# philip-bl/dctn

Hardware: AMD Instinct MI355X
Metric: EPS-contraction windows/sec (fwd+bwd) (higher is better)
Workload: dtype bf16; 1 GPU; cfg2 EPS[(3,4)]+linear bf16 B1024/GPU; parallelism=dp1

## Files before the change

dctn_amd/csrc/eps_mfma.hip:

```cpp
#include "common.h"

#include <cstdlib>
#include <type_traits>

typedef __attribute__((ext_vector_type(8))) __bf16 bf16x8;
typedef __attribute__((ext_vector_type(16))) float f32x16;
typedef __attribute__((ext_vector_type(8))) float f32x8;
typedef __attribute__((ext_vector_type(2))) int int2v;
typedef __attribute__((ext_vector_type(4))) int int4v;
typedef __attribute__((ext_vector_type(2))) float f32x2;

namespace {

constexpr int ilog2(int v) { return v <= 1 ? 0 : 1 + ilog2(v >> 1); }

template <typename S> __device__ __forceinline__ float to_f32(S v) { return (float)v; }

__device__ __forceinline__ float half_sum(float v) {
  const int iv = __float_as_int(v);
  const int2v r = __builtin_amdgcn_permlane32_swap(iv, iv, false, false);
  return __int_as_float(r[0]) + __int_as_float(r[1]);
}

__device__ __forceinline__ void swap_halves(float& a, float& b) {
// ... 20 lines not shown
}

typedef short s16x4 __attribute__((ext_vector_type(4)));
typedef short s16x8 __attribute__((ext_vector_type(8)));
constexpr int LROW = 32;
struct TrLane {
  int wr[4];
  int rd_lo, rd_hi;
};
__device__ __forceinline__ TrLane tr_lane(int lane) {
  TrLane t;
#pragma unroll
  for (int c = 0; c < 4; ++c) t.wr[c] = lane * LROW + (((c + (lane >> 1)) & 3) << 3);
  const int g = lane >> 4, q = (lane >> 2) & 3, pp = lane & 3;
  const int lc = 2 * (g & 1) + (pp >> 1), half = pp & 1;
  const int row = 8 * (g >> 1) + q;
  t.rd_lo = row * LROW + (((lc + (row >> 1)) & 3) << 3) + 4 * half;
  t.rd_hi = (row + 4) * LROW + (((lc + ((row + 4) >> 1)) & 3) << 3) + 4 * half;
  return t;
}
__device__ __forceinline__ bf16x8 tr_frag(const short* tile, int ks, const TrLane& t) {
  typedef __attribute__((address_space(3))) s16x4 lds_s16x4;
  const s16x4 lo = __builtin_amdgcn_ds_read_tr16_b64_v4i16((lds_s16x4*)(tile + t.rd_lo + ks * 16 * LROW));
  const s16x4 hi = __builtin_amdgcn_ds_read_tr16_b64_v4i16((lds_s16x4*)(tile + t.rd_hi + ks * 16 * LROW));
  const s16x8 v = {lo[0], lo[1], lo[2], lo[3], hi[0], hi[1], hi[2], hi[3]};
  return __builtin_bit_cast(bf16x8, v);
}

struct FastDiv {
  unsigned M, s1, s2;
};
__device__ __forceinline__ unsigned fdiv(unsigned n, const FastDiv& d) {
  const unsigned t = __umulhi(d.M, n);
  return (t + ((n - t) >> d.s1)) >> d.s2;
}

#define MFMA_MAXN 16
struct MfmaP {
  int C, B, K, O, Ho, Wo;
  int P;
  int npg;
  int spc, nchunks;
  unsigned foffb[MFMA_MAXN];
  unsigned rowoffb[MFMA_MAXN];
  unsigned s1b, s2b, s3b, s4b;
  unsigned x_bytes;
  unsigned o_bytes, o_s1b;
  FastDiv div_wo;
  int rowvec_ok;
  int vec_ok;
  int Cout;
  unsigned hw_rowb, hw_bytes;
  int ncb;
  int opts;
#ifdef DCTN_STAMPS
  unsigned long long* stamps;
#endif
};

#ifdef DCTN_STAMPS
#define DCTN_STAMP(P, SLOT)                                                                      \
  do {                                                                                           \
    __builtin_amdgcn_sched_barrier(0);                                                           \
    unsigned long long t_;                                                                       \
    asm volatile("s_memrealtime %0\n\ts_waitcnt lgkmcnt(0)" : "=s"(t_)::"memory");               \
    if ((P).stamps && threadIdx.x == 0) (P).stamps[(long long)blockIdx.x * 8 + (SLOT)] = t_;     \
    __builtin_amdgcn_sched_barrier(0);                                                           \
  } while (0)
static unsigned long long* g_stamps = nullptr;
void dctn_stamps_set(unsigned long long* p) { g_stamps = p; }
__device__ unsigned long long* g_dev_stamps = nullptr;
void dctn_reduce_stamps_set(unsigned long long* p) { (void)hipMemcpyToSymbol(HIP_SYMBOL(g_dev_stamps), &p, sizeof(p)); }
#define DCTN_STAMP_T(P, SLOT, TID)                                                              \
  do {                                                                                           \
    __builtin_amdgcn_sched_barrier(0);                                                           \
    unsigned long long t_;                                                                       \
    asm volatile("s_memrealtime %0\n\ts_waitcnt lgkmcnt(0)" : "=s"(t_)::"memory");               \
    if ((P).stamps && threadIdx.x == (TID)) (P).stamps[(long long)blockIdx.x * 8 + (SLOT)] = t_;  \
    __builtin_amdgcn_sched_barrier(0);                                                           \
  } while (0)
#define DCTN_STAMP_ROLE_ROW 1024
#define DCTN_STAMP_R(P, SLOT)                                                                    \
  do {                                                                                           \
    __builtin_amdgcn_sched_barrier(0);                                                           \
    unsigned long long t_;                                                                       \
    asm volatile("s_memrealtime %0\n\ts_waitcnt lgkmcnt(0)" : "=s"(t_)::"memory");               \
    if ((P).stamps && threadIdx.x == 64 * 8)                                                     \
      (P).stamps[(long long)(DCTN_STAMP_ROLE_ROW + blockIdx.x) * 8 + (SLOT)] = t_;               \
    __builtin_amdgcn_sched_barrier(0);                                                           \
  } while (0)
#define DCTN_STAMP_G(SLOT)                                                                       \
  do {                                                                                           \
    __builtin_amdgcn_sched_barrier(0);                                                           \
    unsigned long long t_;                                                                       \
    asm volatile("s_memrealtime %0\n\ts_waitcnt lgkmcnt(0)" : "=s"(t_)::"memory");               \
    if (g_dev_stamps && threadIdx.x == 0) g_dev_stamps[(long long)blockIdx.x * 8 + (SLOT)] = t_;  \
    __builtin_amdgcn_sched_barrier(0);                                                           \
  } while (0)
#else
#define DCTN_STAMP(P, SLOT) do { } while (0)
#define DCTN_STAMP_T(P, SLOT, TID) do { } while (0)
#define DCTN_STAMP_G(SLOT) do { } while (0)
#define DCTN_STAMP_R(P, SLOT) do { } while (0)
#endif

typedef __attribute__((ext_vector_type(4))) unsigned u32x4;
typedef __attribute__((ext_vector_type(2))) unsigned u32x2;
typedef __attribute__((ext_vector_type(2))) __bf16 bf16x2;

__device__ __forceinline__ __amdgpu_buffer_rsrc_t make_rsrc(const void* ptr, unsigned bytes) {
  return __builtin_amdgcn_make_buffer_rsrc(const_cast<void*>(ptr), 0, (int)bytes, 0x00020000);
}

template <typename S, int N, bool VEC, int ROWS>
struct RawWindow {
  u32x4 row[ROWS > 0 ? ROWS : 1];
  unsigned v[(ROWS == 0 && VEC) ? N * (int)(sizeof(S) / 2) : 1];
  unsigned e[(ROWS == 0 && !VEC) ? 2 * N : 1];
};

template <typename S, int N, bool VEC, int ROWS>
__device__ __forceinline__ void issue_window(__amdgpu_buffer_rsrc_t rs, unsigned voff, unsigned soff,
                                             const MfmaP& p, RawWindow<S, N, VEC, ROWS>& raw) {
  if constexpr (ROWS > 0) {
#pragma unroll
    for (int rw = 0; rw < ROWS; ++rw)
      raw.row[rw] = __builtin_amdgcn_raw_buffer_load_b128(rs, voff, soff + p.rowoffb[rw], 0);
  } else if constexpr (VEC) {
#pragma unroll
    for (int n = 0; n < N; ++n) {
      if constexpr (sizeof(S) == 2) {
        raw.v[n] = __builtin_amdgcn_raw_buffer_load_b32(rs, voff, soff + p.foffb[n], 0);
      } else {
        const u32x2 t = __builtin_amdgcn_raw_buffer_load_b64(rs, voff, soff + p.foffb[n], 0);
        raw.v[2 * n] = t.x;
        raw.v[2 * n + 1] = t.y;
      }
    }
  } else {
#pragma unroll
    for (int n = 0; n < N; ++n)
#pragma unroll
      for (int q = 0; q < 2; ++q) {
        if constexpr (sizeof(S) == 2)
          raw.e[2 * n + q] = (unsigned)(unsigned short)__builtin_amdgcn_raw_buffer_load_b16(
              rs, voff, soff + p.foffb[n] + q * p.s4b, 0);
        else
          raw.e[2 * n + q] = __builtin_amdgcn_raw_buffer_load_b32(rs, voff, soff + p.foffb[n] + q * p.s4b, 0);
      }
  }
}

template <typename S, int N, bool VEC, int ROWS>
__device__ __forceinline__ void unpack_window(const RawWindow<S, N, VEC, ROWS>& raw, float (&xv)[N][2]) {
  if constexpr (ROWS > 0) {
    constexpr int KK = N / ROWS;
// ... 94 lines not shown
template <typename S, int OP, bool VEC>
__device__ __forceinline__ void store_row(__amdgpu_buffer_rsrc_t rs, unsigned voff, unsigned soff, int O,
                                          const float (&v)[OP]) {
  constexpr int DW = RawRow<S, OP>::DW;
  if constexpr (VEC) {
    unsigned d[DW];
#pragma unroll
    for (int i = 0; i < DW; ++i)
      d[i] = sizeof(S) == 2 ? pack_bf16(v[2 * i], v[2 * i + 1]) : __float_as_uint(v[i * (OP / DW)]);
    if constexpr (DW == 1) {
      __builtin_amdgcn_raw_buffer_store_b32(d[0], rs, voff, soff, 0);
    } else if constexpr (DW == 2) {
      __builtin_amdgcn_raw_buffer_store_b64(u32x2{d[0], d[1]}, rs, voff, soff, 0);
    } else {
#pragma unroll
      for (int i = 0; i < DW / 4; ++i)
        __builtin_amdgcn_raw_buffer_store_b128(u32x4{d[4 * i], d[4 * i + 1], d[4 * i + 2], d[4 * i + 3]}, rs, voff,
                                               soff + 16u * i, 0);
    }
  } else {
#pragma unroll
    for (int o = 0; o < OP; ++o)
      if (o < O) {
        if constexpr (sizeof(S) == 2)
          __builtin_amdgcn_raw_buffer_store_b16((unsigned short)(pack_bf16(v[o], 0.f) & 0xffffu), rs, voff,
                                                soff + 2u * o, 0);
        else
          __builtin_amdgcn_raw_buffer_store_b32(__float_as_uint(v[o]), rs, voff, soff + 4u * o, 0);
      }
  }
}

struct WaveJob {
  int b0, b1;
  unsigned voff_x;
  unsigned voff_o;
  int pos;
  bool valid;
};
__device__ __forceinline__ WaveJob wave_job(const MfmaP& p, int waves_per_block, int esz, bool grouped = false) {
  const int nb = gridDim.x;
  const int vb = (nb % 8 == 0) ? (int)(blockIdx.x % 8) * (nb / 8) + (int)(blockIdx.x / 8) : (int)blockIdx.x;
  const int wave = __builtin_amdgcn_readfirstlane(vb * waves_per_block + (int)(threadIdx.x >> 6));
  int chunk = wave / p.npg, pg = wave - chunk * p.npg;
  if (grouped) {
    const int cb = vb / p.npg;
    pg = vb - cb * p.npg;
    chunk = __builtin_amdgcn_readfirstlane(cb * waves_per_block + (int)(threadIdx.x >> 6));
    if (cb >= p.ncb) chunk = p.nchunks;
  }
  WaveJob j;
  j.b0 = chunk < p.nchunks ? chunk * p.spc : 0;
  j.b1 = chunk < p.nchunks ? (j.b0 + p.spc < p.B ? j.b0 + p.spc : p.B) : 0;
  j.pos = pg * 64 + (int)(threadIdx.x & 63);
  j.valid = j.pos < p.P;
  const unsigned pu = j.valid ? (unsigned)j.pos : 0u;
  const unsigned ho = fdiv(pu, p.div_wo), wo = pu - ho * (unsigned)p.Wo;
  j.voff_x = j.valid ? ho * p.s2b + wo * p.s3b : p.x_bytes;
  j.voff_o = j.valid ? pu * (unsigned)(p.O * esz) : p.o_bytes;
  return j;
}

template <int N0>
__device__ __forceinline__ void build_p0(const float (*xv)[2], bf16x8 (&X)[(1 << N0) / 16],
                                         bf16x8 (&Y)[(1 << N0) / 16]) {
  constexpr int KS = (1 << N0) / 16;
  const f32x2 x1 = {xv[N0 - 1][0], xv[N0 - 1][1]}, x2 = {xv[N0 - 2][0], xv[N0 - 2][1]};
  const f32x2 m01 = bmul2(xv[N0 - 3][0], x2), m23 = bmul2(xv[N0 - 3][1], x2);
  const f32x2 lo[4] = {bmul2(m01[0], x1), bmul2(m01[1], x1), bmul2(m23[0], x1), bmul2(m23[1], x1)};
#pragma unroll
  for (int s = 0; s < KS; ++s) {
    float hi = 1.f;
#pragma unroll
    for (int t = 0; t < N0 - 4; ++t) hi = t == 0 ? xv[N0 - 5][s & 1] : hi * xv[N0 - 5 - t][(s >> t) & 1];
    const f32x2 x4 = {xv[N0 - 4][0], xv[N0 - 4][1]};
    const f32x2 h = N0 > 4 ? bmul2(hi, x4) : x4;
    int4v rx, ry;
#pragma unroll
    for (int i = 0; i < 4; ++i) {
      const f32x2 a = bmul2(h[0], lo[i]), b = bmul2(h[1], lo[i]);
      rx[i] = (int)pack_bf16(a[0], a[1]);
      ry[i] = (int)pack_bf16(b[0], b[1]);
    }
    X[s] = __builtin_bit_cast(bf16x8, rx);
    Y[s] = __builtin_bit_cast(bf16x8, ry);
  }
}

template <typename S, int N0, int N1, int OP, bool XVEC, bool OVEC, int ROWS>
__global__ __launch_bounds__(256) __attribute__((amdgpu_waves_per_eu(OP <= 4 ? 4 : 2))) void eps_fwd_q2reg_k(const S* __restrict__ x,
                                                       const S* __restrict__ core,
                                                       S* __restrict__ out, double* __restrict__ stats, MfmaP p) {
  constexpr int N = N0 + N1, A = 1 << N0, BN = 1 << N1, KS = A / 16, MT = BN * OP / 32;
  constexpr int LOGO = ilog2(OP);
  static_assert(MT >= 1 && KS >= 1, "tile too small");
  constexpr int TOT = A * BN * OP, PER = TOT / 256;
  static_assert(TOT % 256 == 0, "core staging assumes a multiple of 256 elements");
  __shared__ __attribute__((aligned(16))) bf16_t cs[TOT];
  const int tid = threadIdx.x, lane = tid & 63;
  DCTN_STAMP(p, 0);
  const WaveJob job = wave_job(p, 4, (int)sizeof(S));
  const __amdgpu_buffer_rsrc_t rs_x = make_rsrc(x, p.x_bytes), rs_o = make_rsrc(out, p.o_bytes);
  RawWindow<S, N, XVEC, ROWS> raw;
  if (job.b0 < job.b1) issue_window<S, N, XVEC, ROWS>(rs_x, job.voff_x, (unsigned)job.b0 * p.s1b, p, raw);
  {
    S tmp[PER];
// ... 281 lines not shown
    f32x4v hd = {0.f, 0.f, 0.f, 0.f};
#pragma unroll
    for (int ks = 0; ks < HK; ++ks) {
      const bf16x8 fb = *reinterpret_cast<const bf16x8*>(brd + 32 * ks);
      hd = __builtin_amdgcn_mfma_f32_16x16x32_bf16(wf[ks], fb, hd, 0, 0, 0);
    }
    wave_lds_sync();
    {
      const int sl = lane & 15, cb = 4 * (lane >> 4);
      if (sl < g1 - g0) {
#pragma unroll
        for (int v = 0; v < 4; ++v) hsum[grp & 1][sl][cb + v][wv] = hd[v];
      }
    }
    DCTN_STAMP(p, 3);
    __syncthreads();
    for (int e = tid; e < (g1 - g0) * p.Cout; e += (int)blockDim.x) {
      const int sl = e / p.Cout, c = e - sl * p.Cout;
      float t = (float)bias[c];
      for (int w = 0; w < nwv; ++w) t += hsum[grp & 1][sl][c][w];
      logits[(long long)(g0 + sl) * p.Cout + c] = (bf16_t)t;
    }
  }
  DCTN_STAMP(p, 4);
}

constexpr int HEADT_WAVES = 16;
constexpr int HEADT_GS = 4;
constexpr int HEADT_MAXKS = 6;
constexpr int headt_pitch(int F) { return (F + 31) / 32 * 32 + 8; }

template <int N0, int N1, int OP, int ROWS, bool BLK4>
__global__ __launch_bounds__(64 * HEADT_WAVES) void eps_fwd_head_q2reg_t_k(const bf16_t* __restrict__ x,
                                                                           const bf16_t* __restrict__ core,
                                                                           const bf16_t* __restrict__ hw,
                                                                           const bf16_t* __restrict__ bias,
                                                                           bf16_t* __restrict__ out,
                                                                           bf16_t* __restrict__ logits, MfmaP p) {
  typedef bf16_t S;
  typedef __attribute__((ext_vector_type(4))) float f32x4v;
  constexpr int N = N0 + N1, A = 1 << N0, BN = 1 << N1, KS = A / 16, MT = BN * OP / 32;
  constexpr int LOGO = ilog2(OP);
  constexpr int TOT = A * BN * OP;
  static_assert(OP % 2 == 0 && TOT % 4 == 0, "outputs are handled as bf16 pairs");
  __shared__ __attribute__((aligned(16))) bf16_t cs[TOT];
  __shared__ float hsum[HEADT_WAVES][HEADT_GS][16];
  __shared__ unsigned step_ctr;
  extern __shared__ __attribute__((aligned(16))) short ftile[];
  const int tid = threadIdx.x, lane = tid & 63;
  const int wv = __builtin_amdgcn_readfirstlane(tid >> 6);
  const int b0 = (int)blockIdx.x * p.spc, b1 = b0 + p.spc < p.B ? b0 + p.spc : p.B;
  const int F = p.P * OP, LP = headt_pitch(F);
  const __amdgpu_buffer_rsrc_t rs_x = make_rsrc(x, p.x_bytes), rs_o = make_rsrc(out, p.o_bytes);
  for (int e0 = 0; e0 < TOT; e0 += 4 * 64 * HEADT_WAVES) {
    S tmp[4];
#pragma unroll
    for (int i = 0; i < 4; ++i) {
      const int ec = e0 + tid + i * 64 * HEADT_WAVES, e = ec < TOT ? ec : TOT - 1, o = e % OP, ab = e / OP;
      tmp[i] = core[(long long)ab * p.O + (o < p.O ? o : 0)];
    }
#pragma unroll
    for (int i = 0; i < 4; ++i) {
      const int e = e0 + tid + i * 64 * HEADT_WAVES, o = e % OP, ab = e / OP, bb = ab % BN, aa = ab / BN;
      const int code = ((bb >> 1) << LOGO) | o;
      const int row = (((code >> 2) & 3) << 3) | ((bb & 1) << 2) | (code & 3);
      const int dst = ((((code >> 4) * KS + (aa >> 4)) * 64 + ((aa >> 3) & 1) * 32 + row) << 3) | (aa & 7);
      if (e < TOT) cs[dst] = o < p.O ? tmp[i] : (bf16_t)0.f;
    }
  }
  for (int e = tid; e < HEADT_GS * (LP - F); e += 64 * HEADT_WAVES) ftile[(e / (LP - F)) * LP + F + e % (LP - F)] = 0;
  __syncthreads();
  bf16x8 cf[MT][KS];
#pragma unroll
  for (int t = 0; t < MT; ++t)
#pragma unroll
    for (int s = 0; s < KS; ++s)
      cf[t][s] = *reinterpret_cast<const bf16x8*>(&cs[((t * KS + s) * 64 + lane) * 8]);

  auto lane_at = [&](int pg, bool live, unsigned& voff_x, unsigned& voff_o, int& pos) {
    pos = pg * 64 + lane;
    const bool valid = live && pos < p.P;
    const unsigned pu = (unsigned)(pos < p.P ? pos : p.P - 1);
    const unsigned ho = fdiv(pu, p.div_wo), wo = pu - ho * (unsigned)p.Wo;
    voff_x = valid ? ho * p.s2b + wo * p.s3b : p.x_bytes;
    voff_o = valid ? pu * (unsigned)(OP * 2) : p.o_bytes;
  };
  auto draw = [&]() {
    unsigned v = 0;
    if (lane == 0) v = __hip_atomic_fetch_add(&step_ctr, 1u, __ATOMIC_RELAXED, __HIP_MEMORY_SCOPE_WORKGROUP);
    return (int)__builtin_amdgcn_readfirstlane(v);
  };

  for (int g0 = b0; g0 < b1; g0 += HEADT_GS) {
    const int ng = g0 + HEADT_GS < b1 ? HEADT_GS : b1 - g0;
    const int nsteps = ng * p.npg;
    if (tid == 0) step_ctr = 2 * HEADT_WAVES;
    __syncthreads();
    int cur = wv, nxt = wv + HEADT_WAVES;
    int s = cur / p.npg, pg = cur - s * p.npg, pos;
    unsigned voff_x, voff_o;
    lane_at(pg, cur < nsteps, voff_x, voff_o, pos);
    RawWindow<S, N, true, ROWS> raw;
    issue_window<S, N, true, ROWS>(rs_x, voff_x, (unsigned)(g0 + (cur < nsteps ? s : 0)) * p.s1b, p, raw);
    while (cur < nsteps) {
      float xv[N][2];
      unpack_window<S, N, true, ROWS>(raw, xv);
      const unsigned vo = voff_o, so = (unsigned)(g0 + s) * p.o_s1b;
      short* trow = ftile + s * LP + (pos < p.P ? pos : 0) * OP;
      const bool tvalid = pos < p.P;
      {
        cur = nxt;
        s = cur / p.npg;
        pg = cur - s * p.npg;
        lane_at(pg, cur < nsteps, voff_x, voff_o, pos);
        issue_window<S, N, true, ROWS>(rs_x, voff_x, (unsigned)(g0 + (cur < nsteps ? s : 0)) * p.s1b, p, raw);
        nxt = draw();
        __builtin_amdgcn_sched_barrier(0);
      }
      bf16x8 pf0[KS], pf1[KS];
      build_p0<N0>(xv, pf0, pf1);
#pragma unroll
      for (int s2 = 0; s2 < KS; ++s2) swap_halves(pf0[s2], pf1[s2]);
      float m0[BN / 2], m1[BN / 2];
      {
        float ph[BN / 2];
        ph[0] = xv[N - 2][0];
        ph[1] = xv[N - 2][1];
#pragma unroll
        for (int u = 2; u < N1; ++u)
#pragma unroll
          for (int bh = (1 << (u - 1)) - 1; bh >= 0; --bh) {
            const f32x2 pr = bmul2(ph[bh], f32x2{xv[N - 1 - u][0], xv[N - 1 - u][1]});
            ph[bh] = pr[0];
            ph[bh | (1 << (u - 1))] = pr[1];
          }
#pragma unroll
        for (int bh = 0; bh < BN / 2; ++bh) {
          const f32x2 mm = bmul2(ph[bh], f32x2{xv[N - 1][0], xv[N - 1][1]});
          m0[bh] = mm[0];
          m1[bh] = mm[1];
          swap_halves(m0[bh], m1[bh]);
        }
      }
      float res0[OP], res1[OP];
#pragma unroll
      for (int o = 0; o < OP; ++o) { res0[o] = 0.f; res1[o] = 0.f; }
#pragma unroll
      for (int t = 0; t < MT; ++t) {
#pragma unroll
        for (int set = 0; set < 2; ++set) {
          f32x16 acc;
#pragma unroll
          for (int v = 0; v < 16; ++v) acc[v] = 0.f;
#pragma unroll
          for (int s2 = 0; s2 < KS; ++s2)
            acc = __builtin_amdgcn_mfma_f32_32x32x16_bf16(cf[t][s2], set ? pf1[s2] : pf0[s2], acc, 0, 0, 0);
#pragma unroll
          for (int v = 0; v < 16; v += 2) {
            const int code = (t << 4) | ((v >> 2) << 2) | (v & 3);
            const float mm = set ? m1[code >> LOGO] : m0[code >> LOGO];
            float* dst = set ? res1 : res0;
            const int o = code & (OP - 1);
            const f32x2 r = __builtin_elementwise_fma(f32x2{mm, mm}, f32x2{acc[v], acc[v + 1]}, f32x2{dst[o], dst[o + 1]});
            dst[o] = r[0];
            dst[o + 1] = r[1];
          }
        }
      }
      unsigned pk[OP / 2];
#pragma unroll
      for (int i = 0; i < OP / 2; ++i) {
        float a0 = res0[2 * i], a1 = res1[2 * i], c0 = res0[2 * i + 1], c1 = res1[2 * i + 1];
        swap_halves(a0, a1);
        swap_halves(c0, c1);
        pk[i] = pack_bf16(a0 + a1, c0 + c1);
      }
      if constexpr (OP == 2) {
        if constexpr (!BLK4) __builtin_amdgcn_raw_buffer_store_b32(pk[0], rs_o, vo, so, 0);
        if (tvalid) *reinterpret_cast<unsigned*>(trow) = pk[0];
      } else if constexpr (OP == 4) {
        if constexpr (!BLK4) __builtin_amdgcn_raw_buffer_store_b64(u32x2{pk[0], pk[1]}, rs_o, vo, so, 0);
        if (tvalid) *reinterpret_cast<u32x2*>(trow) = u32x2{pk[0], pk[1]};
      } else {
#pragma unroll
        for (int i = 0; i < OP / 8; ++i) {
          const u32x4 q = u32x4{pk[4 * i], pk[4 * i + 1], pk[4 * i + 2], pk[4 * i + 3]};
          if constexpr (!BLK4) __builtin_amdgcn_raw_buffer_store_b128(q, rs_o, vo, so + 16u * i, 0);
          if (tvalid) *reinterpret_cast<u32x4*>(trow + 8 * i) = q;
        }
      }
    }
    const int nks = (F + 31) / 32;
    const int c = lane & 15, kg = lane >> 4;
    const __amdgpu_buffer_rsrc_t rs_hw = make_rsrc(hw, p.hw_bytes);
    u32x4 wf[HEADT_MAXKS];
#pragma unroll
    for (int i = 0; i < HEADT_MAXKS; ++i) {
      const int ks = wv + HEADT_WAVES * i, k = 32 * ks + 8 * kg;
      const unsigned vo2 = (ks < nks && c < p.Cout && k + 7 < F) ? (unsigned)c * p.hw_rowb + (unsigned)k * 2u : p.hw_bytes;
      wf[i] = __builtin_amdgcn_raw_buffer_load_b128(rs_hw, vo2, 0, 0);
    }
    __syncthreads();
    f32x4v hd = {0.f, 0.f, 0.f, 0.f};
    const short* brd = ftile + (c < HEADT_GS ? c : HEADT_GS - 1) * LP + 8 * kg;
#pragma unroll
    for (int i = 0; i < HEADT_MAXKS; ++i) {
      const int ks = wv + HEADT_WAVES * i;
      if (ks < nks) {
        const bf16x8 fb = *reinterpret_cast<const bf16x8*>(brd + 32 * ks);
        hd = __builtin_amdgcn_mfma_f32_16x16x32_bf16(__builtin_bit_cast(bf16x8, wf[i]), fb, hd, 0, 0, 0);
      }
    }
    if (c < HEADT_GS) {
#pragma unroll
      for (int v = 0; v < 4; ++v) hsum[wv][c][4 * kg + v] = hd[v];
    }
    if constexpr (BLK4) {
      static_assert(HEADT_GS == 4, "a group is one block of the blocked4 layout");
      const unsigned sob = (unsigned)(g0 >> 2) * (unsigned)F * 8u;
      for (int f = 2 * tid; f < F; f += 2 * 64 * HEADT_WAVES) {
        unsigned r[HEADT_GS];
#pragma unroll
        for (int i = 0; i < HEADT_GS; ++i) r[i] = i < ng ? *reinterpret_cast<const unsigned*>(ftile + i * LP + f) : 0u;
        const u32x4 q = u32x4{__builtin_amdgcn_perm(r[1], r[0], 0x05040100u), __builtin_amdgcn_perm(r[3], r[2], 0x05040100u),
                              __builtin_amdgcn_perm(r[1], r[0], 0x07060302u), __builtin_amdgcn_perm(r[3], r[2], 0x07060302u)};
        __builtin_amdgcn_raw_buffer_store_b128(q, rs_o, (unsigned)f * 8u, sob, 0);
      }
    }
    __syncthreads();
    if (tid < HEADT_GS * 16) {
      const int sl = tid >> 4, cc = tid & 15;
      if (sl < ng && cc < p.Cout) {
        float t = (float)bias[cc];
#pragma unroll
        for (int w = 0; w < HEADT_WAVES; ++w) t += hsum[w][sl][cc];
        logits[(long long)(g0 + sl) * p.Cout + cc] = (bf16_t)t;
      }
    }
  }
}

constexpr int BWD_WAVES = 8;
constexpr size_t dcore_dyn_lds_bytes(int mt) { return (size_t)BWD_WAVES * (1 + mt) * 64 * 32 * sizeof(short); }

__device__ __forceinline__ void head_dw_role_waves(const bf16_t* __restrict__ feat, const bf16_t* __restrict__ dL,
                                                   bf16_t* __restrict__ dW, int B, int Cout, long long F, int n_dw,
                                                   int rw, float* __restrict__ lds, const MfmaP& p);
template <typename S, int N0, int N1, int OP, bool XVEC, bool OVEC, int ROWS, int HEADC, int DWROLE = 0>
__global__ __launch_bounds__(64 * (BWD_WAVES + DWROLE)) void eps_bwd_dcore_q2reg_k(const S* __restrict__ x,
                                                             const S* __restrict__ dY,
                                                             const S* __restrict__ hw,
                                                             const S* __restrict__ feat,
                                                             float* __restrict__ partial,
                                                             float* __restrict__ dwpart, MfmaP p,
                                                             S* __restrict__ dW, int n_dw) {
  constexpr int N = N0 + N1, A = 1 << N0, BN = 1 << N1, KS = A / 16, MT = BN * OP / 32;
  constexpr int AT = A >= 32 ? A / 32 : 1;
  constexpr int LOGO = ilog2(OP);
  constexpr bool LDST = A == 32 && MT <= 2;
  __shared__ float red[BWD_WAVES][32 * 32];
  extern __shared__ __attribute__((aligned(16))) unsigned char dsm[];
  const int tid = threadIdx.x, lane = tid & 63, r = lane & 31, h = lane >> 5, wv = tid >> 6;
  DCTN_STAMP(p, 0);
  if constexpr (DWROLE > 0) {
    static_assert(HEADC > 0 && HEADC <= 16 && LDST && OVEC && XVEC && sizeof(S) == 2 && OP == 4, "the dW role rides the HEADMM path");
    const int rw = __builtin_amdgcn_readfirstlane(wv) - BWD_WAVES;
    if (rw >= 0) {
      head_dw_role_waves(feat, dY, dW, p.B, p.Cout, (long long)p.P * OP, n_dw, rw,
                         reinterpret_cast<float*>(dsm + dcore_dyn_lds_bytes(MT) + 8192), p);
      return;
    }
#ifdef DCTN_DWROLE_PRIO
    __builtin_amdgcn_s_setprio(DCTN_DWROLE_PRIO);
#endif
  }
  short* tiles = reinterpret_cast<short*>(dsm) + wv * ((1 + MT) * 64 * LROW);
  const TrLane trl = tr_lane(lane);

  bf16x8 ident[2];
#pragma unroll
  for (int sp = 0; sp < 2; ++sp)
#pragma unroll
    for (int j = 0; j < 8; ++j) ident[sp][j] = (bf16_t)((16 * sp + 8 * h + j == r) ? 1.f : 0.f);

  f32x16 acc[MT][AT];
#pragma unroll
  for (int t = 0; t < MT; ++t)
#pragma unroll
    for (int a = 0; a < AT; ++a)
#pragma unroll
      for (int v = 0; v < 16; ++v) acc[t][a][v] = 0.f;

// ... 41 lines not shown
      for (int s2 = 0; s2 < KS; ++s2) {
        *reinterpret_cast<bf16x8*>(tiles + trl.wr[2 * s2]) = X[s2];
        *reinterpret_cast<bf16x8*>(tiles + trl.wr[2 * s2 + 1]) = Y[s2];
      }
      float dyl[OP];
      make_dy(dyl);
#pragma unroll
      for (int t = 0; t < MT; ++t)
#pragma unroll
        for (int c4 = 0; c4 < 4; ++c4) {
          int4v zr;
#pragma unroll
          for (int jp = 0; jp < 4; ++jp) {
            const int m = (t << 5) | (c4 << 3) | (2 * jp);
            static_assert(OP >= 2, "a pair of consecutive m shares b = m >> LOGO");
            const f32x2 zz = bmul2(p1[m >> LOGO], f32x2{dyl[m & (OP - 1)], dyl[(m + 1) & (OP - 1)]});
            zr[jp] = (int)pack_bf16(zz[0], zz[1]);
          }
          *reinterpret_cast<bf16x8*>(tiles + (1 + t) * 64 * LROW + trl.wr[c4]) = __builtin_bit_cast(bf16x8, zr);
        }
      wave_lds_sync();
#pragma unroll
      for (int ks = 0; ks < 4; ++ks) {
        const bf16x8 p0t = tr_frag(tiles, ks, trl);
#pragma unroll
        for (int t = 0; t < MT; ++t) {
          const bf16x8 zt = tr_frag(tiles + (1 + t) * 64 * LROW, ks, trl);
          acc[t][0] = __builtin_amdgcn_mfma_f32_32x32x16_bf16(zt, p0t, acc[t][0], 0, 0, 0);
        }
      }
    }
  };
  if constexpr (HEADMM) {
    static_assert(BWD_WAVES * 64 * 16 == 16 * 64 * OP * 2, "one 16-byte load per thread stages the weight slice");
    RawWindow<S, N, XVEC, ROWS> rawm;
    if (job.b0 < job.b1) issue_window<S, N, XVEC, ROWS>(rs_x, job.voff_x, (unsigned)job.b0 * p.s1b, p, rawm);
    const unsigned dl_bytes = (unsigned)p.B * (unsigned)p.Cout * 2u, dlrow = (unsigned)p.Cout * 2u;
    const __amdgpu_buffer_rsrc_t rs_dl = make_rsrc(dY, dl_bytes);
    const int slot = 4 * (r >> 3) + (r & 3);
    const bool rlow = ((r >> 2) & 1) == 0;
    u32x4 fa;
    auto issue_group = [&](int g0) {
      const unsigned voff_a = (r < 16 && g0 + slot < job.b1 && 8 * h < p.Cout) ? (unsigned)slot * dlrow + 16u * h : dl_bytes;
      fa = __builtin_amdgcn_raw_buffer_load_b128(rs_dl, voff_a, (unsigned)g0 * dlrow, 0);
    };
    u32x4 wv4;
    {
      const __amdgpu_buffer_rsrc_t rs_hw = make_rsrc(hw, p.hw_bytes);
      const int e = 2 * tid, c = e >> 6, posl = e & 63, pos = job.pos - lane + posl;
      const unsigned voff = pos < p.P ? (unsigned)pos * (unsigned)(OP * 2) : p.hw_bytes;
      wv4 = __builtin_amdgcn_raw_buffer_load_b128(rs_hw, voff, (unsigned)c * p.hw_rowb, 0);
      if (pos + 1 >= p.P) { wv4.z = 0u; wv4.w = 0u; }
    }
    *reinterpret_cast<u32x4*>(dsm + dcore_dyn_lds_bytes(MT) + (size_t)tid * 16) = wv4;
    __syncthreads();
    const unsigned* wlds = reinterpret_cast<const unsigned*>(dsm + dcore_dyn_lds_bytes(MT));
    DCTN_STAMP(p, 1);
    for (int g0 = job.b0; g0 < job.b1; g0 += 8) {
      issue_group(g0);
      f32x8 dyg[OP];
      auto group_products = [&]() {
        int4v a0, a1;
#pragma unroll
        for (int d = 0; d < 4; ++d) {
          const bool dv = 8 * h + 2 * d < p.Cout;
          const int v = (int)(d == 0 ? fa.x : d == 1 ? fa.y : d == 2 ? fa.z : fa.w);
          a0[d] = (dv && rlow) ? v : 0;
          a1[d] = (dv && !rlow) ? v : 0;
        }
        int4v bw[OP][2];
#pragma unroll
        for (int o = 0; o < OP; ++o) {
          const unsigned sel = (o & 1) ? 0x07060302u : 0x05040100u;
#pragma unroll
          for (int hh = 0; hh < 2; ++hh)
#pragma unroll
            for (int d = 0; d < 4; ++d) {
              const unsigned lo = wlds[((8 * h + 2 * d) * 64 + 32 * hh + r) * 2 + (o >> 1)];
              const unsigned hi = wlds[((8 * h + 2 * d + 1) * 64 + 32 * hh + r) * 2 + (o >> 1)];
              bw[o][hh][d] = (int)__builtin_amdgcn_perm(hi, lo, sel);
            }
        }
        __builtin_amdgcn_sched_barrier(0);
#pragma unroll
        for (int o = 0; o < OP; ++o) {
          f32x16 dya;
#pragma unroll
          for (int v = 0; v < 16; ++v) dya[v] = 0.f;
#pragma unroll
          for (int hh = 0; hh < 2; ++hh)
            dya = __builtin_amdgcn_mfma_f32_32x32x16_bf16(__builtin_bit_cast(bf16x8, hh == 0 ? a0 : a1),
                                                           __builtin_bit_cast(bf16x8, bw[o][hh]), dya, 0, 0, 0);
          dyg[o] = __builtin_shufflevector(dya, dya, 0, 1, 2, 3, 4, 5, 6, 7);
        }
        __builtin_amdgcn_sched_barrier(0);
        asm volatile("s_nop 7\n\ts_nop 7" ::"v"(a0), "v"(a1), "v"(bw[0][0]), "v"(bw[0][1]), "v"(bw[1][0]), "v"(bw[1][1]),
                     "v"(bw[2 % OP][0]), "v"(bw[2 % OP][1]), "v"(bw[3 % OP][0]), "v"(bw[3 % OP][1]) : "memory");
        __builtin_amdgcn_sched_barrier(0);
      };
      group_products();
#pragma unroll
      for (int sidx = 0; sidx < 8; ++sidx) {
        const int b = g0 + sidx;
        if (b < job.b1) {
          float xv[N][2];
          unpack_window<S, N, XVEC, ROWS>(rawm, xv);
          {
            const int bn = b + 1 < job.b1 ? b + 1 : b;
            issue_window<S, N, XVEC, ROWS>(rs_x, job.voff_x, (unsigned)bn * p.s1b, p, rawm);
            __builtin_amdgcn_sched_barrier(0);
          }
          ldst_step(xv, [&](float (&dyo)[OP]) {
// ... 102 lines not shown
        p0t[set][a][0] = pack8(d[0], d[1], d[2], d[3], d[4], d[5], d[6], d[7]);
        p0t[set][a][1] = pack8(d[8], d[9], d[10], d[11], d[12], d[13], d[14], d[15]);
      }
    float p1[BN];
    p1[0] = xv[N - 1][0];
    p1[1] = xv[N - 1][1];
#pragma unroll
    for (int u = 1; u < N1; ++u)
#pragma unroll
      for (int b = (1 << u) - 1; b >= 0; --b) {
        const float lo = p1[b];
        p1[b | (1 << u)] = lo * xv[N - 1 - u][1];
        p1[b] = lo * xv[N - 1 - u][0];
      }
#pragma unroll
    for (int t = 0; t < MT; ++t) {
      bf16x8 zf[2][2];
#pragma unroll
      for (int sp = 0; sp < 2; ++sp) {
        float za[8], zb[8];
#pragma unroll
        for (int j = 0; j < 8; ++j) {
          const int ma = (t << 5) | (sp << 4) | j;
          const int mb = ma | 8;
          za[j] = p1[ma >> LOGO] * dy[ma & (OP - 1)];
          zb[j] = p1[mb >> LOGO] * dy[mb & (OP - 1)];
        }
        zf[0][sp] = pack8(za[0], za[1], za[2], za[3], za[4], za[5], za[6], za[7]);
        zf[1][sp] = pack8(zb[0], zb[1], zb[2], zb[3], zb[4], zb[5], zb[6], zb[7]);
        swap_halves(zf[0][sp], zf[1][sp]);
      }
#pragma unroll
      for (int set = 0; set < 2; ++set) {
        f32x16 d;
#pragma unroll
        for (int v = 0; v < 16; ++v) d[v] = 0.f;
#pragma unroll
        for (int sp = 0; sp < 2; ++sp)
          d = __builtin_amdgcn_mfma_f32_32x32x16_bf16(zf[set][sp], ident[sp], d, 0, 0, 0);
        bf16x8 zt[2];
        zt[0] = pack8(d[0], d[1], d[2], d[3], d[4], d[5], d[6], d[7]);
        zt[1] = pack8(d[8], d[9], d[10], d[11], d[12], d[13], d[14], d[15]);
#pragma unroll
        for (int a = 0; a < AT; ++a)
#pragma unroll
          for (int s2 = 0; s2 < 2; ++s2)
            acc[t][a] = __builtin_amdgcn_mfma_f32_32x32x16_bf16(zt[s2], p0t[set][a][s2], acc[t][a], 0, 0, 0);
      }
    }
  }
  }

  DCTN_STAMP(p, 3);
  float* dst = partial + (long long)blockIdx.x * (MT * 32) * (AT * 32);
  if constexpr (LDST) {
    static_assert(AT == 1 && (size_t)BWD_WAVES * MT * 1024 * 4 <= dcore_dyn_lds_bytes(MT), "dCore tiles must fit");
    float* big = reinterpret_cast<float*>(dsm);
    DCTN_STAMP_T(p, 6, 64 * (BWD_WAVES - 1));
    __syncthreads();
    DCTN_STAMP(p, 7);
#pragma unroll
    for (int t = 0; t < MT; ++t)
#pragma unroll
      for (int v = 0; v < 16; ++v) {
        const int row = (v & 3) + 8 * (v >> 2) + 4 * h;
        big[(wv * MT + t) * 1024 + row * 32 + r] = acc[t][0][v];
      }
    __syncthreads();
    for (int e = tid; e < MT * 1024; e += 64 * BWD_WAVES) {
      float sum = 0.f;
#pragma unroll
      for (int k = 0; k < BWD_WAVES; ++k) sum += big[k * MT * 1024 + e];
      dst[e] = sum;
    }
  } else {
#pragma unroll
    for (int t = 0; t < MT; ++t)
#pragma unroll
      for (int a = 0; a < AT; ++a) {
        __syncthreads();
#pragma unroll
        for (int v = 0; v < 16; ++v) {
          const int row = (v & 3) + 8 * (v >> 2) + 4 * h;
          red[wv][row * 32 + r] = acc[t][a][v];
        }
        __syncthreads();
        for (int e = tid; e < 1024; e += 64 * BWD_WAVES) {
          float sum = 0.f;
#pragma unroll
          for (int k = 0; k < BWD_WAVES; ++k) sum += red[k][e];
          const int row = e >> 5, col = e & 31;
          dst[(long long)(t * 32 + row) * (AT * 32) + a * 32 + col] = sum;
        }
      }
  }

  DCTN_STAMP(p, 4);
  if constexpr (HEADC > 0 && !HEADMM) {
    constexpr int SLOT = LDST ? (int)(dcore_dyn_lds_bytes(MT) / (BWD_WAVES * 4)) : 1024;
    constexpr int CPR_RAW = SLOT / (64 * OP);
    constexpr int CPR = CPR_RAW > HEADC ? HEADC : CPR_RAW;
    float* red1 = LDST ? reinterpret_cast<float*>(dsm) : &red[0][0];
    const int nbk = gridDim.x;
    const int vbk = (nbk % 8 == 0) ? (int)(blockIdx.x % 8) * (nbk / 8) + (int)(blockIdx.x / 8) : (int)blockIdx.x;
    const int cb = vbk / p.npg, pg = vbk - cb * p.npg;
    const int F = p.P * OP;
// ... 393 lines not shown
      ext += (dims[i] - 1) * p.s[i];
    }
    if ((ext + 1) * esz >= (1LL << 31)) return false;
    if (p.Wn * p.O * esz >= (1LL << 31)) return false;
  }
  const int op = next_pow2(p.O);
  return op >= 2 ? op <= 16 : true;
}

FastDiv make_fastdiv(unsigned d) {
  FastDiv f;
  if (d <= 1) {
    f.M = 0; f.s1 = 0; f.s2 = 0;
    return f;
  }
  unsigned l = 0;
  while ((1ull << l) < d) ++l;
  f.M = (unsigned)(((1ull << 32) * ((1ull << l) - d)) / d + 1);
  f.s1 = 1;
  f.s2 = l - 1;
  return f;
}

void fill_mp(MfmaP& m, const EpsP& p, const void* x, int dtype) {
  const long long esz = dtype == DCTN_BF16 ? 2 : 4;
  for (int n = 0; n < p.N && n < MFMA_MAXN; ++n) {
    const int pos = n / p.C, ch = n - pos * p.C;
    const int dh = pos / p.K, dw = pos - dh * p.K;
    m.foffb[n] = (unsigned)((ch * p.s[0] + dh * p.s[2] + dw * p.s[3]) * esz);
  }
  m.s1b = (unsigned)(p.s[1] * esz); m.s2b = (unsigned)(p.s[2] * esz);
  m.s3b = (unsigned)(p.s[3] * esz); m.s4b = (unsigned)(p.s[4] * esz);
  long long ext = 0;
  const long long dims[5] = {p.C, p.B, p.H, p.W, p.Q};
  for (int i = 0; i < 5; ++i) ext += (dims[i] - 1) * p.s[i];
  m.x_bytes = (unsigned)((ext + 1) * esz);
  const int rows = p.K * p.C;
  for (int rw = 0; rw < MFMA_MAXN; ++rw) m.rowoffb[rw] = 0;
  for (int rw = 0; rw < rows && rw < MFMA_MAXN; ++rw) {
    const int dh = rw / p.C, ch = rw - dh * p.C;
    m.rowoffb[rw] = (unsigned)((ch * p.s[0] + dh * p.s[2]) * esz);
  }
  m.rowvec_ok = dtype == DCTN_BF16 && p.s[4] == 1 && p.s[3] == 2 && p.K <= 4 && rows <= MFMA_MAXN / 2 &&
                ((p.N == 9 && rows == 3) || (p.N == 8 && rows == 4));
  m.div_wo = make_fastdiv((unsigned)p.Wo);
  m.C = p.C; m.B = p.B; m.K = p.K; m.O = p.O; m.Ho = p.Ho; m.Wo = p.Wo;
  m.P = p.Ho * p.Wo;
  m.npg = (m.P + 63) / 64;
  m.spc = 1; m.nchunks = p.B;
  m.o_s1b = (unsigned)((long long)m.P * p.O * esz);
  m.o_bytes = (unsigned)(p.Wn * p.O * esz);
  m.vec_ok = p.s[4] == 1 && p.s[0] % 2 == 0 && p.s[1] % 2 == 0 && p.s[2] % 2 == 0 &&
             p.s[3] % 2 == 0 && ((uintptr_t)x % 4) == 0;
  m.Cout = 0; m.hw_rowb = 0; m.hw_bytes = 0; m.ncb = 0;
  m.opts = p.opts;
#ifdef DCTN_STAMPS
  m.stamps = g_stamps;
#endif
}

constexpr int FWD_BLOCKS_PER_CU = 4;

template <int N0, int N1, int OP>
constexpr size_t dcore_dyn_lds() {
  constexpr int A = 1 << N0, MT = (1 << N1) * OP / 32;
  return (A == 32 && MT <= 2) ? (size_t)BWD_WAVES * (1 + MT) * 64 * LROW * sizeof(short) : 0;
}
#define DCTN_DCORE_LAUNCH(KERNEL, G, B, DYN, ST, ...)                                                  \
  do {                                                                                                 \
    if ((DYN) > 0 && !dctn_lds_optin((const void*)KERNEL, DYN)) return DCTN_ERR_UNSUPPORTED;       \
    hipLaunchKernelGGL(KERNEL, G, B, DYN, ST, __VA_ARGS__);                                            \
  } while (0)

int plan_waves(MfmaP& m, int wpb, long long target) {
  long long chunks = target / m.npg;
  if (chunks < 1) chunks = 1;
  if (chunks > m.B) chunks = m.B;
  m.spc = (int)((m.B + chunks - 1) / chunks);
  m.nchunks = (m.B + m.spc - 1) / m.spc;
  const long long waves = (long long)m.nchunks * m.npg;
  long long blocks = (waves + wpb - 1) / wpb;
  if (blocks >= 8) blocks = (blocks + 7) / 8 * 8;
  return (int)blocks;
}

template <typename S>
bool row_vec_ok(const MfmaP& m, int OP, const void* ptr) {
  return m.O == OP && ((uintptr_t)ptr % 4) == 0 && (OP * sizeof(S)) % 4 == 0;
}

template <typename S, int N0, int N1, int OP>
int fwd_launch_t(const void* x, const void* core, void* out, double* stats, const MfmaP& m_in, hipStream_t st) {
  MfmaP m = m_in;
  const int blocks = plan_waves(m, 4, (long long)FWD_BLOCKS_PER_CU * dctn_dev().cus * 4);
  const bool ovec = out == nullptr || row_vec_ok<S>(m, OP, out);
  const dim3 g((unsigned)blocks), b(256);
  constexpr int NN = N0 + N1;
  constexpr int RW = NN == 9 ? 3 : 4;
  if (m.rowvec_ok && m.vec_ok && ovec && sizeof(S) == 2)
    hipLaunchKernelGGL((eps_fwd_q2reg_k<S, N0, N1, OP, true, true, RW>), g, b, 0, st, (const S*)x,
                       (const S*)core, (S*)out, stats, m);
  else if (m.vec_ok && ovec)
    hipLaunchKernelGGL((eps_fwd_q2reg_k<S, N0, N1, OP, true, true, 0>), g, b, 0, st, (const S*)x,
                       (const S*)core, (S*)out, stats, m);
  else if (m.vec_ok)
    hipLaunchKernelGGL((eps_fwd_q2reg_k<S, N0, N1, OP, true, false, 0>), g, b, 0, st, (const S*)x,
                       (const S*)core, (S*)out, stats, m);
  else
    hipLaunchKernelGGL((eps_fwd_q2reg_k<S, N0, N1, OP, false, false, 0>), g, b, 0, st, (const S*)x,
                       (const S*)core, (S*)out, stats, m);
  DCTN_CHECK_LAUNCH();
  dctn_set_last_kernel("eps_fwd_mfma_q2reg");
  return DCTN_OK;
}

template <typename S, int N0, int N1, int OP>
int bwd_launch_t(const void* x, const void* dY, void* dCore, void* ws, const MfmaP& m_in,
                 hipStream_t st) {
  constexpr int A = 1 << N0, BN = 1 << N1, AT = A >= 32 ? A / 32 : 1;
  constexpr size_t DYN = dcore_dyn_lds<N0, N1, OP>();
  MfmaP m = m_in;
  const int grid = plan_waves(m, BWD_WAVES, (long long)dctn_dev().cus * BWD_WAVES);
  const bool ovec = row_vec_ok<S>(m, OP, dY);
  const dim3 g(grid), b(64 * BWD_WAVES);
  constexpr int NN = N0 + N1;
  constexpr int RW = NN == 9 ? 3 : 4;
  if (m.rowvec_ok && m.vec_ok && ovec && sizeof(S) == 2)
    DCTN_DCORE_LAUNCH((eps_bwd_dcore_q2reg_k<S, N0, N1, OP, true, true, RW, 0>), g, b, DYN, st,
                       (const S*)x, (const S*)dY, (const S*)nullptr, (const S*)nullptr, (float*)ws, (float*)nullptr, m, (S*)nullptr, 0);
  else if (m.vec_ok && ovec)
    DCTN_DCORE_LAUNCH((eps_bwd_dcore_q2reg_k<S, N0, N1, OP, true, true, 0, 0>), g, b, DYN, st,
                       (const S*)x, (const S*)dY, (const S*)nullptr, (const S*)nullptr, (float*)ws, (float*)nullptr, m, (S*)nullptr, 0);
  else if (m.vec_ok)
    DCTN_DCORE_LAUNCH((eps_bwd_dcore_q2reg_k<S, N0, N1, OP, true, false, 0, 0>), g, b, DYN, st,
                       (const S*)x, (const S*)dY, (const S*)nullptr, (const S*)nullptr, (float*)ws, (float*)nullptr, m, (S*)nullptr, 0);
  else
    DCTN_DCORE_LAUNCH((eps_bwd_dcore_q2reg_k<S, N0, N1, OP, false, false, 0, 0>), g, b, DYN, st,
                       (const S*)x, (const S*)dY, (const S*)nullptr, (const S*)nullptr, (float*)ws, (float*)nullptr, m, (S*)nullptr, 0);
  DCTN_CHECK_LAUNCH();
  if (m.opts & DCTN_OPT_MAIN_KERNEL_ONLY) return DCTN_PARTIAL;
  hipLaunchKernelGGL((eps_bwd_dcore_reduce_k<S>), dim3(BN * OP * AT), dim3(256), 0, st,
                     (const float*)ws, (S*)dCore, grid, A, BN, m.O, OP, AT * 32);
  DCTN_CHECK_LAUNCH();
  dctn_set_last_kernel("eps_bwd_mfma_q2reg");
  return DCTN_OK;
}

int plan_grouped(MfmaP& m) {
  if (m.npg > dctn_dev().cus) return 0;
  long long ncb = dctn_dev().cus / m.npg;
  const long long need = (m.B + BWD_WAVES - 1) / BWD_WAVES;
  if (ncb > need) ncb = need;
  m.spc = (int)((m.B + ncb * BWD_WAVES - 1) / (ncb * BWD_WAVES));
  m.nchunks = (m.B + m.spc - 1) / m.spc;
  m.ncb = (m.nchunks + BWD_WAVES - 1) / BWD_WAVES;
  long long blocks = (long long)m.ncb * m.npg;
  if (blocks >= 8) blocks = (blocks + 7) / 8 * 8;
  return blocks <= dctn_dev().cus ? (int)blocks : 0;
}

size_t head_dw_partial_bytes(const EpsP& p, int Cout) {
  const long long P = (long long)p.Ho * p.Wo, npg = (P + 63) / 64;
  if (npg > dctn_dev().cus) return 0;
  return (size_t)(dctn_dev().cus / npg) * ((size_t)Cout * (size_t)(P * p.O) + 16) * sizeof(float);
}

long long blocked4_bytes(const MfmaP& m) { return (long long)(m.B + 3) / 4 * 4 * m.P * m.O * 2; }
template <int N0, int N1, int OP>
bool head_blocked4_ok(const MfmaP& m) {
  constexpr int A = 1 << N0, MT = (1 << N1) * OP / 32;
  const long long F = (long long)m.P * OP;
  return A == 32 && MT <= 2 && OP == 4 && m.vec_ok && blocked4_bytes(m) < (1LL << 31) && !(m.opts & DCTN_OPT_SMALL_CHUNKS) &&
         F % 8 == 0 && F <= (long long)HEADT_WAVES * HEADT_MAXKS * 32;
}

template <int N0, int N1, int OP>
int bwd_head_launch_t(const void* x, const void* dL, const void* hw, const void* feat, void* dCore, void* dW,
                      void* dBias, void* ws, size_t core_ws_bytes, const MfmaP& m_in, hipStream_t st) {
  typedef bf16_t S;
  constexpr int A = 1 << N0, BN = 1 << N1, AT = A >= 32 ? A / 32 : 1;
  constexpr size_t DYN = dcore_dyn_lds<N0, N1, OP>();
  MfmaP m = m_in;
  const bool blk = (m.opts & DCTN_OPT_HEAD_FEATURES_BLOCKED4) != 0;
  if (m.O != OP || m.Cout < 2 || m.Cout > 16 || m.Cout % 2 != 0) return DCTN_ERR_UNSUPPORTED;
  if (((uintptr_t)dL % 4) != 0 || ((uintptr_t)hw % 4) != 0 || ((uintptr_t)feat % (blk ? 16 : 4)) != 0) return DCTN_ERR_UNSUPPORTED;
  if (blk && !head_blocked4_ok<N0, N1, OP>(m)) return DCTN_ERR_UNSUPPORTED;
  const int grid = plan_grouped(m);
  if (grid == 0) return DCTN_ERR_UNSUPPORTED;
  float* dwpart = reinterpret_cast<float*>(static_cast<unsigned char*>(ws) + core_ws_bytes);
  const long long nW = (long long)m.Cout * m.P * OP;
  constexpr int MT = BN * OP / 32;
  const bool headmm = A == 32 && MT <= 2 && OP == 4 && m.vec_ok;
  if (headmm && (long long)m.B * m.P * OP * 2 >= (1LL << 31)) return DCTN_ERR_UNSUPPORTED;
  const bool gemm = headmm;

  const dim3 g(grid), b(64 * BWD_WAVES);
  constexpr int NN = N0 + N1;
  constexpr int RW = NN == 9 ? 3 : 4;
  const int n_slices = (int)(((long long)m.P * OP + DWG_BFW - 1) / DWG_BFW);
  bool dwrole = false;
  if constexpr (A == 32 && MT <= 2 && OP == 4) {
    constexpr size_t RDYN = DYN + 8192 + DWR_LDS_BYTES;
#define DCTN_HEAD_ROLE_LAUNCH(ROWSV, HC)                                                                          \
  do {                                                                                                            \
    const void* kfn = (const void*)eps_bwd_dcore_q2reg_k<S, N0, N1, OP, true, true, ROWSV, HC, DWR_WAVES>;        \
    if (dctn_lds_optin(kfn, RDYN)) {                                                                              \
      hipLaunchKernelGGL((eps_bwd_dcore_q2reg_k<S, N0, N1, OP, true, true, ROWSV, HC, DWR_WAVES>), g,             \
                         dim3(64 * (BWD_WAVES + DWR_WAVES)), RDYN, st, (const S*)x, (const S*)dL, (const S*)hw,   \
                         (const S*)feat, (float*)ws, dwpart, m, (S*)dW, dW ? n_slices : 0);                       \
      dwrole = true;                                                                                              \
    }                                                                                                             \
  } while (0)
    if (blk && headmm) {
      if (m.rowvec_ok) {
        if (m.Cout <= 10) DCTN_HEAD_ROLE_LAUNCH(RW, 10); else DCTN_HEAD_ROLE_LAUNCH(RW, 16);
      } else {
        if (m.Cout <= 10) DCTN_HEAD_ROLE_LAUNCH(0, 10); else DCTN_HEAD_ROLE_LAUNCH(0, 16);
      }
    }
#undef DCTN_HEAD_ROLE_LAUNCH
  }
#define DCTN_HEAD_LAUNCH(XV, ROWSV, HC)                                                                        \
  DCTN_DCORE_LAUNCH((eps_bwd_dcore_q2reg_k<S, N0, N1, OP, XV, true, ROWSV, HC>), g, b, (DYN > 0 ? DYN + 8192 : 0), st, (const S*)x, \
                     (const S*)dL, (const S*)hw, (const S*)feat, (float*)ws, dwpart, m, (S*)nullptr, 0)
  if (dwrole) {
  } else if (m.rowvec_ok && m.vec_ok) {
    if (m.Cout <= 10) DCTN_HEAD_LAUNCH(true, RW, 10); else DCTN_HEAD_LAUNCH(true, RW, 16);
  } else if (m.vec_ok) {
    if (m.Cout <= 10) DCTN_HEAD_LAUNCH(true, 0, 10); else DCTN_HEAD_LAUNCH(true, 0, 16);
  } else {
    if (m.Cout <= 10) DCTN_HEAD_LAUNCH(false, 0, 10); else DCTN_HEAD_LAUNCH(false, 0, 16);
  }
#undef DCTN_HEAD_LAUNCH
  DCTN_CHECK_LAUNCH();
  if (m.opts & DCTN_OPT_MAIN_KERNEL_ONLY) return DCTN_PARTIAL;
  const int fw = blk ? DWG_BFW : DWG_FW;
  const int n_core = BN * OP * AT;
  if (dwrole) {
    hipLaunchKernelGGL(eps_head_reduce_k, dim3(n_core + 1), dim3(1024), 0, st, (const float*)ws, (S*)dCore, grid, A, BN, m.O, OP,
                       AT * 32, n_core, (const float*)dwpart, (S*)nullptr, m.ncb, nW, 0, (const S*)dL, (S*)dBias, m.B, m.Cout,
                       (const S*)feat, 0);
    DCTN_CHECK_LAUNCH();
    dctn_set_last_kernel("eps_head_bwd_mfma_q2reg");
    return DCTN_OK;
  }
  const int n_dw = gemm ? (int)(((long long)m.P * OP + fw - 1) / fw) : (int)((nW + 255) / 256);
  const size_t gemm_lds = (size_t)DWG_WAVES * (fw / 4) * 64 * sizeof(float);
// ... 164 lines not shown
```

Measured before the change: 27.69 billion windows/s.

## Skew per-wave sample counts in grouped dCore backward and reorder head stores

In the grouped backward dCore kernel, the first half of the waves in a block now take more samples and the second half fewer (skew = spc/3). This is meant to balance against the dW role waves that share the CU, or to stagger when waves finish. The first sample group's load is now issued before the LDS weight staging and barrier, to hide its latency. In the head forward kernel, the bias is prefetched into LDS and the blocked4 feature store is moved ahead of the MFMA head reduction. Stamp probes are also added. The skew risks load imbalance if the waves are not actually asymmetric.

```diff
diff --git a/dctn_amd/csrc/eps_mfma.hip b/dctn_amd/csrc/eps_mfma.hip
--- a/dctn_amd/csrc/eps_mfma.hip
+++ b/dctn_amd/csrc/eps_mfma.hip
@@ -96,6 +96,7 @@
   int Cout;
   unsigned hw_rowb, hw_bytes;
   int ncb;
+  int skew;
   int opts;
 #ifdef DCTN_STAMPS
   unsigned long long* stamps;
@@ -133,6 +134,16 @@
       (P).stamps[(long long)(DCTN_STAMP_ROLE_ROW + blockIdx.x) * 8 + (SLOT)] = t_;               \
     __builtin_amdgcn_sched_barrier(0);                                                           \
   } while (0)
+#define DCTN_STAMP_WAVE_ROW 1536
+#define DCTN_STAMP_W(P, WV)                                                                      \
+  do {                                                                                           \
+    __builtin_amdgcn_sched_barrier(0);                                                           \
+    unsigned long long t_;                                                                       \
+    asm volatile("s_memrealtime %0\n\ts_waitcnt lgkmcnt(0)" : "=s"(t_)::"memory");               \
+    if ((P).stamps && (threadIdx.x & 63) == 0 && (WV) < 8)                                        \
+      (P).stamps[(long long)(DCTN_STAMP_WAVE_ROW + blockIdx.x) * 8 + (WV)] = t_;                 \
+    __builtin_amdgcn_sched_barrier(0);                                                           \
+  } while (0)
 #define DCTN_STAMP_G(SLOT)                                                                       \
   do {                                                                                           \
     __builtin_amdgcn_sched_barrier(0);                                                           \
@@ -146,6 +157,7 @@
 #define DCTN_STAMP_T(P, SLOT, TID) do { } while (0)
 #define DCTN_STAMP_G(SLOT) do { } while (0)
 #define DCTN_STAMP_R(P, SLOT) do { } while (0)
+#define DCTN_STAMP_W(P, WV) do { } while (0)
 #endif
 
 typedef __attribute__((ext_vector_type(4))) unsigned u32x4;
@@ -346,6 +358,15 @@
   WaveJob j;
   j.b0 = chunk < p.nchunks ? chunk * p.spc : 0;
   j.b1 = chunk < p.nchunks ? (j.b0 + p.spc < p.B ? j.b0 + p.spc : p.B) : 0;
+  if (grouped && p.skew > 0) {
+    const int w = __builtin_amdgcn_readfirstlane((int)(threadIdx.x >> 6)), half = waves_per_block / 2;
+    const int n_old = p.spc + p.skew, n_young = p.spc - p.skew;
+    const int s0 = (vb / p.npg) * waves_per_block * p.spc + (w < half ? w * n_old : half * n_old + (w - half) * n_young);
+    const int s1 = s0 + (w < half ? n_old : n_young);
+    const bool live = vb / p.npg < p.ncb && s0 < p.B;
+    j.b0 = live ? s0 : 0;
+    j.b1 = live ? (s1 < p.B ? s1 : p.B) : 0;
+  }
   j.pos = pg * 64 + (int)(threadIdx.x & 63);
   j.valid = j.pos < p.P;
   const unsigned pu = j.valid ? (unsigned)j.pos : 0u;
@@ -733,6 +754,9 @@
   const int b0 = (int)blockIdx.x * p.spc, b1 = b0 + p.spc < p.B ? b0 + p.spc : p.B;
   const int F = p.P * OP, LP = headt_pitch(F);
   const __amdgpu_buffer_rsrc_t rs_x = make_rsrc(x, p.x_bytes), rs_o = make_rsrc(out, p.o_bytes);
+  __shared__ float bias_s[16];
+  DCTN_STAMP(p, 0);
+  float bias_v = 0.f;
   for (int e0 = 0; e0 < TOT; e0 += 4 * 64 * HEADT_WAVES) {
     S tmp[4];
 #pragma unroll
@@ -740,6 +764,7 @@
       const int ec = e0 + tid + i * 64 * HEADT_WAVES, e = ec < TOT ? ec : TOT - 1, o = e % OP, ab = e / OP;
       tmp[i] = core[(long long)ab * p.O + (o < p.O ? o : 0)];
     }
+    if (e0 == 0 && wv == 0) bias_v = (float)bias[(lane & 15) < p.Cout ? (lane & 15) : 0];
 #pragma unroll
     for (int i = 0; i < 4; ++i) {
       const int e = e0 + tid + i * 64 * HEADT_WAVES, o = e % OP, ab = e / OP, bb = ab % BN, aa = ab / BN;
@@ -749,6 +774,7 @@
       if (e < TOT) cs[dst] = o < p.O ? tmp[i] : (bf16_t)0.f;
     }
   }
+  if (wv == 0) bias_s[lane & 15] = bias_v;
   for (int e = tid; e < HEADT_GS * (LP - F); e += 64 * HEADT_WAVES) ftile[(e / (LP - F)) * LP + F + e % (LP - F)] = 0;
   __syncthreads();
   bf16x8 cf[MT][KS];
@@ -757,6 +783,7 @@
 #pragma unroll
     for (int s = 0; s < KS; ++s)
       cf[t][s] = *reinterpret_cast<const bf16x8*>(&cs[((t * KS + s) * 64 + lane) * 8]);
+  DCTN_STAMP(p, 1);
 
   auto lane_at = [&](int pg, bool live, unsigned& voff_x, unsigned& voff_o, int& pos) {
     pos = pg * 64 + lane;
@@ -783,6 +810,9 @@
     lane_at(pg, cur < nsteps, voff_x, voff_o, pos);
     RawWindow<S, N, true, ROWS> raw;
     issue_window<S, N, true, ROWS>(rs_x, voff_x, (unsigned)(g0 + (cur < nsteps ? s : 0)) * p.s1b, p, raw);
+#ifdef DCTN_STAMPS
+    bool first_step = true;
+#endif
     while (cur < nsteps) {
       float xv[N][2];
       unpack_window<S, N, true, ROWS>(raw, xv);
@@ -870,7 +900,13 @@
           if (tvalid) *reinterpret_cast<u32x4*>(trow + 8 * i) = q;
         }
       }
-    }
+#ifdef DCTN_STAMPS
+      if (first_step) DCTN_STAMP(p, 2);
+      first_step = false;
+#endif
+    }
+    DCTN_STAMP(p, 3);
+    DCTN_STAMP_T(p, 4, 64 * (HEADT_WAVES - 1));
     const int nks = (F + 31) / 32;
     const int c = lane & 15, kg = lane >> 4;
     const __amdgpu_buffer_rsrc_t rs_hw = make_rsrc(hw, p.hw_bytes);
@@ -882,6 +918,20 @@
       wf[i] = __builtin_amdgcn_raw_buffer_load_b128(rs_hw, vo2, 0, 0);
     }
     __syncthreads();
+    DCTN_STAMP(p, 5);
+    if constexpr (BLK4) {
+      static_assert(HEADT_GS == 4, "a group is one block of the blocked4 layout");
+      const unsigned sob = (unsigned)(g0 >> 2) * (unsigned)F * 8u;
+      for (int f = 2 * tid; f < F; f += 2 * 64 * HEADT_WAVES) {
+        unsigned r[HEADT_GS];
+#pragma unroll
+        for (int i = 0; i < HEADT_GS; ++i) r[i] = i < ng ? *reinterpret_cast<const unsigned*>(ftile + i * LP + f) : 0u;
+        const u32x4 q = u32x4{__builtin_amdgcn_perm(r[1], r[0], 0x05040100u), __builtin_amdgcn_perm(r[3], r[2], 0x05040100u),
+                              __builtin_amdgcn_perm(r[1], r[0], 0x07060302u), __builtin_amdgcn_perm(r[3], r[2], 0x07060302u)};
+        __builtin_amdgcn_raw_buffer_store_b128(q, rs_o, (unsigned)f * 8u, sob, 0);
+      }
+    }
+    __builtin_amdgcn_sched_barrier(0);
     f32x4v hd = {0.f, 0.f, 0.f, 0.f};
     const short* brd = ftile + (c < HEADT_GS ? c : HEADT_GS - 1) * LP + 8 * kg;
 #pragma unroll
@@ -896,29 +946,18 @@
 #pragma unroll
       for (int v = 0; v < 4; ++v) hsum[wv][c][4 * kg + v] = hd[v];
     }
-    if constexpr (BLK4) {
-      static_assert(HEADT_GS == 4, "a group is one block of the blocked4 layout");
-      const unsigned sob = (unsigned)(g0 >> 2) * (unsigned)F * 8u;
-      for (int f = 2 * tid; f < F; f += 2 * 64 * HEADT_WAVES) {
-        unsigned r[HEADT_GS];
-#pragma unroll
-        for (int i = 0; i < HEADT_GS; ++i) r[i] = i < ng ? *reinterpret_cast<const unsigned*>(ftile + i * LP + f) : 0u;
-        const u32x4 q = u32x4{__builtin_amdgcn_perm(r[1], r[0], 0x05040100u), __builtin_amdgcn_perm(r[3], r[2], 0x05040100u),
-                              __builtin_amdgcn_perm(r[1], r[0], 0x07060302u), __builtin_amdgcn_perm(r[3], r[2], 0x07060302u)};
-        __builtin_amdgcn_raw_buffer_store_b128(q, rs_o, (unsigned)f * 8u, sob, 0);
-      }
-    }
     __syncthreads();
     if (tid < HEADT_GS * 16) {
       const int sl = tid >> 4, cc = tid & 15;
       if (sl < ng && cc < p.Cout) {
-        float t = (float)bias[cc];
+        float t = bias_s[cc];
 #pragma unroll
         for (int w = 0; w < HEADT_WAVES; ++w) t += hsum[w][sl][cc];
         logits[(long long)(g0 + sl) * p.Cout + cc] = (bf16_t)t;
       }
     }
   }
+  DCTN_STAMP(p, 6);
 }
 
 constexpr int BWD_WAVES = 8;
@@ -1066,12 +1105,13 @@
       wv4 = __builtin_amdgcn_raw_buffer_load_b128(rs_hw, voff, (unsigned)c * p.hw_rowb, 0);
       if (pos + 1 >= p.P) { wv4.z = 0u; wv4.w = 0u; }
     }
+    issue_group(job.b0);
     *reinterpret_cast<u32x4*>(dsm + dcore_dyn_lds_bytes(MT) + (size_t)tid * 16) = wv4;
     __syncthreads();
     const unsigned* wlds = reinterpret_cast<const unsigned*>(dsm + dcore_dyn_lds_bytes(MT));
     DCTN_STAMP(p, 1);
     for (int g0 = job.b0; g0 < job.b1; g0 += 8) {
-      issue_group(g0);
+      if (g0 != job.b0) issue_group(g0);
       f32x8 dyg[OP];
       auto group_products = [&]() {
         int4v a0, a1;
@@ -1280,6 +1320,7 @@
   }
 
   DCTN_STAMP(p, 3);
+  DCTN_STAMP_W(p, wv);
   float* dst = partial + (long long)blockIdx.x * (MT * 32) * (AT * 32);
   if constexpr (LDST) {
     static_assert(AT == 1 && (size_t)BWD_WAVES * MT * 1024 * 4 <= dcore_dyn_lds_bytes(MT), "dCore tiles must fit");
@@ -1779,7 +1820,7 @@
   m.o_bytes = (unsigned)(p.Wn * p.O * esz);
   m.vec_ok = p.s[4] == 1 && p.s[0] % 2 == 0 && p.s[1] % 2 == 0 && p.s[2] % 2 == 0 &&
              p.s[3] % 2 == 0 && ((uintptr_t)x % 4) == 0;
-  m.Cout = 0; m.hw_rowb = 0; m.hw_bytes = 0; m.ncb = 0;
+  m.Cout = 0; m.hw_rowb = 0; m.hw_bytes = 0; m.ncb = 0; m.skew = 0;
   m.opts = p.opts;
 #ifdef DCTN_STAMPS
   m.stamps = g_stamps;
@@ -1873,6 +1914,10 @@
   return DCTN_OK;
 }
 
+#ifndef DCTN_DCORE_SKEW
+#define DCTN_DCORE_SKEW(spc) ((spc) / 3)
+#endif
+
 int plan_grouped(MfmaP& m) {
   if (m.npg > dctn_dev().cus) return 0;
   long long ncb = dctn_dev().cus / m.npg;
@@ -1920,6 +1965,8 @@
   const bool headmm = A == 32 && MT <= 2 && OP == 4 && m.vec_ok;
   if (headmm && (long long)m.B * m.P * OP * 2 >= (1LL << 31)) return DCTN_ERR_UNSUPPORTED;
   const bool gemm = headmm;
+  m.skew = headmm ? DCTN_DCORE_SKEW(m.spc) : 0;
+  if (m.skew >= m.spc) m.skew = m.spc - 1;
 
   const dim3 g(grid), b(64 * BWD_WAVES);
   constexpr int NN = N0 + N1;
```

New measurement: 28.20 billion windows/s, median of 6. +1.8%, better.
